# douglasbagnall/recur

Measured on AMD Instinct MI355X. Metric: BPTT timesteps*streams/sec at 1024-hidden/256-stream, higher is better.
Workload: dtype f32; 1 GPU; text-predict multi-tap generation: hidden 1024, 256 streams/GPU, BPTT depth 20, 42 symbols, RELU, weighted momentum, lr 1e-5; streams_per_gpu=256, global_streams=256, scaling_mode=weak, parallelism=single GPU, rccl_ranks=0, exchange=none

## Files before the change

### recur_amd/csrc/k_common.h

```cpp
#pragma once
#include <hip/hip_runtime.h>
#include <cstring>
#include <utility>
#include <type_traits>
#include <stdint.h>
#include <stdio.h>
#include <stdlib.h>
#include <math.h>
#include "ramd_internal.h"
#include "k_tiles.h"

#define HIP_CHECK(x)                                                              \
  do {                                                                            \
    hipError_t e_ = (x);                                                          \
    if (e_ != hipSuccess) {                                                       \
      fprintf(stderr, "librecur_amd: HIP error %s at %s:%d\n", hipGetErrorString(e_), \
              __FILE__, __LINE__);                                                \
      abort();                                                                    \
    }                                                                             \
  } while (0)

static inline void ramd_check_launch(const char *file, int line) {
  hipError_t e_ = hipGetLastError();
  if (e_ != hipSuccess) {
// ... 464 lines not shown
      const bool keep = s0 + i * 32 < hw.nrows && am[i] != 0;
#pragma unroll
      for (int rr = 0; rr < HO_HR; rr++) {
        const float x = keep ? hv[i][rr] : 0.0f;
        acc[rr].x += x * e4[i].x;
        acc[rr].y += x * e4[i].y;
        acc[rr].z += x * e4[i].z;
        acc[rr].w += x * e4[i].w;
      }
    }
  }
}
struct HoApply {
  float *w, *m;
  float rate, momentum, mw;
};
template <int HO_HR, int BATCH>
__device__ __forceinline__ void chain_ho_delta(const View &v, const HoWork &hw, float *lds, int rank, HoApply ap = HoApply{}) {
  const RamdShape &s = v.sh;
  const int H = s.H, O = s.O, OQ = O >> 2;
  const int HR = (H + hw.workers - 1) / hw.workers;
  const int tid = threadIdx.x, lane = tid & 63, wave = tid >> 6, q4 = lane & 15, gl = lane >> 4;
  const int h0 = rank * HR;
  float4 acc[HO_HR];
#pragma unroll
  for (int rr = 0; rr < HO_HR; rr++) acc[rr] = zero4();
  if (h0 < H) {
    const int q4c = q4 < OQ ? q4 : 0;
    if (hw.active) chain_ho_sum<true, HO_HR, BATCH>(v, hw, h0, HR, q4c, 4 * wave + gl, acc);
    else chain_ho_sum<false, HO_HR, BATCH>(v, hw, h0, HR, q4c, 4 * wave + gl, acc);
#pragma unroll
    for (int rr = 0; rr < HO_HR; rr++) {
      acc[rr].x += __shfl_xor(acc[rr].x, 16, 64); acc[rr].x += __shfl_xor(acc[rr].x, 32, 64);
      acc[rr].y += __shfl_xor(acc[rr].y, 16, 64); acc[rr].y += __shfl_xor(acc[rr].y, 32, 64);
      acc[rr].z += __shfl_xor(acc[rr].z, 16, 64); acc[rr].z += __shfl_xor(acc[rr].z, 32, 64);
      acc[rr].w += __shfl_xor(acc[rr].w, 16, 64); acc[rr].w += __shfl_xor(acc[rr].w, 32, 64);
    }
    if (gl == 0) {
#pragma unroll
      for (int rr = 0; rr < HO_HR; rr++) *reinterpret_cast<float4 *>(lds + 4 * ((wave * HO_HR + rr) * 16 + q4)) = acc[rr];
    }
  }
  const bool fin = tid < HO_HR * 16 && (tid >> 4) < HR && h0 + (tid >> 4) < H && (tid & 15) < OQ;
  const size_t fin_off = fin ? (size_t)(h0 + (tid >> 4)) * O + 4 * (tid & 15) : 0;
  float4 W4 = zero4(), M4 = zero4();
  if (fin && ap.w) {
    W4 = ld4(ap.w + fin_off);
    M4 = ld4(ap.m + fin_off);
  }
  __syncthreads();
  if (fin) {
    const int rr = tid >> 4, q = tid & 15;
    float4 sum = *reinterpret_cast<const float4 *>(lds + 4 * (rr * 16 + q));
    for (int w = 1; w < 8; w++) {
      const float4 t = *reinterpret_cast<const float4 *>(lds + 4 * ((w * HO_HR + rr) * 16 + q));
      sum.x += t.x; sum.y += t.y; sum.z += t.z; sum.w += t.w;
    }
    *reinterpret_cast<float4 *>(hw.dst + fin_off) = sum;
    if (ap.w) {
      float wv[4] = {W4.x, W4.y, W4.z, W4.w}, mv[4] = {M4.x, M4.y, M4.z, M4.w};
      const float dv[4] = {sum.x, sum.y, sum.z, sum.w};
#pragma unroll
      for (int i = 0; i < 4; i++) {
        const float t = dv[i] * ap.rate, mm = mv[i];
        wv[i] += t + mm * ap.mw;
        mv[i] = (mm + t) * ap.momentum;
      }
      *reinterpret_cast<float4 *>(ap.w + fin_off) = make_float4(wv[0], wv[1], wv[2], wv[3]);
      *reinterpret_cast<float4 *>(ap.m + fin_off) = make_float4(mv[0], mv[1], mv[2], mv[3]);
    }
  }
  __syncthreads();
}


struct XcWork {
  int on;
  int row0;
  int nx, nxp;
  const unsigned char *active;
  unsigned flags;
  int done;
  int dense;
};
RAMD_LOCAL int ramd_chain_steps(hipStream_t st, const View &v, const RamdShape *sh, const RamdBuffers *b,
                                int row0, int nrows, HoWork *ho, XcWork *xc);
```

### recur_amd/csrc/k_extras.h

```cpp
#pragma once
#include "k_common.h"
#ifndef XC_STAMP
#define XC_STAMP(i) do { } while (0)
#endif

template <int MAXQ> struct ExtrasIn {
  float4 ev[MAXQ];
  float xi, pv;
};
typedef unsigned u32x4_t __attribute__((ext_vector_type(4)));
template <int MAXQ>
__device__ __forceinline__ void extras_load(const View &v, int t, int r, int nx, int tn, int lane,
                                            ExtrasIn<MAXQ> &in) {
  const RamdShape &s = v.sh;
  const float *erow = v.b.ehi + (t * s.Scap + r) * s.I;
  const float *x = input_row_auto(v, r, t);
  const int nq = (s.H / 4 + 63) / 64;
  const int last4 = s.H / 4 - 1;
#pragma unroll
  for (int i = 0; i < MAXQ; i++) {
    const int k4 = lane + 64 * i;
    const float4 e = ld4(erow + 4 * min(k4, last4));
    in.ev[i] = (i < nq && k4 <= last4) ? e : zero4();
  }
// ... 127 lines not shown
  for (int k0 = 0; k0 < D; k0 += 64) {
    int k = k0 + lane;
    float es = (k < D) ? es_src[(size_t)k * es_stride] : 0.0f;
    bool stop = k < D && (es <= min_error_sum || es > max_error_sum);
    unsigned long long hit = __ballot(stop);
    int last = hit ? __ffsll((long long)hit) - 1 : min(63, D - 1 - k0);
    error_sum = __shfl(es, last, 64);
    if (hit) {
      n_exec = k0 + last + 1;
      break;
    }
  }
  bool broke = n_exec < D || (error_sum <= min_error_sum || error_sum > max_error_sum);
  int t = broke ? D - n_exec + 1 : 0;
  float scale;
  if (error_sum > error_sum_ceiling) {
    scale = soft_clip_dev(error_sum, max_error_sum);
  } else {
    scale = 1.0f;
    if (flags & 64u) {
      int depth_error = D / 4 - t;
      if (mef < MAX_MIN_ERROR_FACTOR_F && (min_error_gain != min_error_sum || depth_error < 0)) {
        mef = (float)((double)mef * (1.0 + depth_error * 1e-3));
      }
      mef = (mef >= ABS_MIN_ERROR_FACTOR_F) ? mef : ABS_MIN_ERROR_FACTOR_F;
    }
  }
  if (lane == 0) {
    as_global(v.b.mef)[r] = mef;
    as_global(v.b.ih_scale)[r] = scale;
    as_global(v.b.bptt_err)[r] = error_sum;
    as_global(v.b.n_exec)[r] = n_exec;
    as_global(v.b.depth_log)[r] = D - t;
    as_global(v.b.stat_depth)[r] = ci.depth_total + (double)(D - t);
  }
  const float cf = (flags & RAMD_IH_SCALE_IN_RATE) ? 1.0f : scale;
  for (int k = lane; k < D; k += 64) as_global(v.b.coef)[(size_t)k * s.Scap + r] = (k < n_exec) ? cf : 0.0f;
}


template <int MAXQ, int THREADS>
__device__ __forceinline__ void extras_control_stream(const View &v, int r, int j, int nx, int nxp, int tn,
                                                      const unsigned char *active, unsigned flags,
                                                      float *es_sh) {
  const RamdShape &s = v.sh;
  const int wave = threadIdx.x >> 6, lane = threadIdx.x & 63;
  const int items = tn == 0 ? s.D + 1 : s.D;
  float *hs_sh = es_sh + s.D;
  ExtrasIn<MAXQ> cur, nxt;
  ControlIn ci = {0.0f, 0.0f, 1.0f, 0.0, true};
  if (wave == 0) ci = bptt_control_load(v, r, j, active);
  if (wave < items) extras_load<MAXQ>(v, wave, r, nx, tn, lane, cur);
  for (int t = wave; t < items; t += THREADS / 64) {
    const int tnext = t + THREADS / 64;
    if (tnext < items) extras_load<MAXQ>(v, tnext, r, nx, tn, lane, nxt);
    if (tn == 0) {
      const float hs = row_sumsq<MAXQ>(cur);
      if (lane == 0) hs_sh[t] = hs;
    }
    if (t < s.D) {
      float es = extras_compute<MAXQ>(v, t, r, nx, nxp, tn, lane, cur);
      if (lane == 0) {
        if (tn != 0) v.b.esum[(size_t)t * s.Scap + r] = es;
        es_sh[t] = es;
      }
    }
    cur = nxt;
  }
  __syncthreads();
  if (wave == 0) {
    if (tn == 0) {
      for (int k = lane; k < s.D; k += 64) {
        const float es = hs_sh[k + 1] + es_sh[k];
        es_sh[k] = es;
        v.b.esum[(size_t)k * s.Scap + r] = es;
      }
      __builtin_amdgcn_s_waitcnt(0xc07f);
    }
    bptt_control_wave(v, r, j, lane, ci, flags, es_sh, 1);
  }
}

constexpr int XT_B = 3, XT_BL = 2;
struct TailPre {
  float xi[XT_B][2];
  ControlIn ci;
};
__device__ __forceinline__ void tail_items(int wave, int NW, int D, int &t0, int &stride, int &t_end) {
  const int NE = NW / 2;
  const int first_late = D > NE * XT_BL ? D - NE * XT_BL : 0;
  stride = NE;
  if (wave < NE) {
    t0 = wave;
    t_end = first_late;
  } else {
    t0 = first_late + (wave - NE);
    t_end = D;
  }
}
template <int THREADS>
__device__ __forceinline__ TailPre extras_tail_prefetch(const View &v, int r, int j, int nx, const unsigned char *active) {
  const RamdShape &s = v.sh;
  constexpr int NW = THREADS / 64;
  const int wave = __builtin_amdgcn_readfirstlane((int)(threadIdx.x >> 6)), lane = threadIdx.x & 63;
  const int D = s.D;
  TailPre p;
  p.ci = ControlIn{0.0f, 0.0f, 1.0f, 0.0, true};
  if (wave == 0) p.ci = bptt_control_load(v, r, j, active);
  const int xcol[2] = {(lane == 0 || lane >= nx) ? 0 : s.hidden_size + lane, lane + 64 < nx ? s.hidden_size + lane + 64 : 0};
  int t0, stride, t_end;
  tail_items(wave, NW, D, t0, stride, t_end);
#pragma unroll
  for (int b = 0; b < XT_B; b++) {
    const int t = t0 + stride * b;
    const auto *x = as_global(input_row<true>(v, r, t < D ? t : D - 1));
#pragma unroll
    for (int h = 0; h < 2; h++) p.xi[b][h] = x[xcol[h]];
  }
  return p;
}

template <int MAXQ, int THREADS, class WaitLast>
__device__ __forceinline__ void extras_control_tail(const View &v, int r, int j, int nx, int nxp,
                                                    const unsigned char *active, unsigned flags, float *es_sh,
                                                    const TailPre *pre, WaitLast &&wait_last) {
  constexpr int B = XT_B;
  const RamdShape &s = v.sh;
  constexpr int NW = THREADS / 64;
  const int wave = __builtin_amdgcn_readfirstlane((int)(threadIdx.x >> 6)), lane = threadIdx.x & 63;
  const int D = s.D;
  float *hs_sh = es_sh + D;
  const int nq = (s.H / 4 + 63) / 64, last4 = s.H / 4 - 1;
  ControlIn ci = {0.0f, 0.0f, 1.0f, 0.0, true};
  if (pre) ci = pre->ci;
  else if (wave == 0) ci = bptt_control_load(v, r, j, active);
  const __amdgpu_buffer_rsrc_t rs = __builtin_amdgcn_make_buffer_rsrc((void *)v.b.ehi, 0, 0x7fffffff, 0x00020000);
  const int xcol[2] = {(lane == 0 || lane >= nx) ? 0 : s.hidden_size + lane, lane + 64 < nx ? s.hidden_size + lane + 64 : 0};
  const unsigned xmask[2] = {lane < nx ? 0xffffffffu : 0u, lane + 64 < nx ? 0xffffffffu : 0u};
  unsigned koff[MAXQ];
  float km[MAXQ];
#pragma unroll
  for (int i = 0; i < MAXQ; i++) {
    const int k4 = lane + 64 * i;
    koff[i] = 16u * (unsigned)min(k4, last4);
    km[i] = (i < nq && k4 <= last4) ? 1.0f : 0.0f;
  }
  auto load_row = [&](int plane, float4 (&e)[MAXQ]) {
    const unsigned row_off = (unsigned)((plane * s.Scap + r) * s.I) * 4u;
#pragma unroll
    for (int i = 0; i < MAXQ; i++) {
      const u32x4_t q = __builtin_amdgcn_raw_buffer_load_b128(rs, (int)(row_off + koff[i]), 0, 16 );
      e[i] = make_float4(__uint_as_float(q.x), __uint_as_float(q.y), __uint_as_float(q.z), __uint_as_float(q.w));
    }
  };
  auto mask_row = [&](float4 (&e)[MAXQ]) {
#pragma unroll
    for (int i = 0; i < MAXQ; i++) { e[i].x *= km[i]; e[i].y *= km[i]; e[i].z *= km[i]; e[i].w *= km[i]; }
  };
  XC_STAMP(3);
  constexpr int NE = NW / 2;
  auto batch = [&](auto BC, const int tb, const int t_stride, const int t_end, const float (*xpre)[2]) {
    constexpr int BB = decltype(BC)::value;
    float xi[BB][2];
    float4 ev[BB][MAXQ], wh[BB][MAXQ], w0[MAXQ];
#pragma unroll
    for (int b = 0; b < BB; b++) {
      if (xpre) {
        xi[b][0] = __uint_as_float(__float_as_uint(xpre[b][0]) & xmask[0]);
        xi[b][1] = __uint_as_float(__float_as_uint(xpre[b][1]) & xmask[1]);
      } else {
        const int t = tb + t_stride * b;
        const auto *x = as_global(input_row<true>(v, r, t < D ? t : D - 1));
#pragma unroll
        for (int h = 0; h < 2; h++) xi[b][h] = __uint_as_float(__float_as_uint(x[xcol[h]]) & xmask[h]);
      }
    }
#pragma unroll
    for (int i = 0; i < MAXQ; i++) w0[i] = ld4g(reinterpret_cast<const char *>(v.b.ih_w) + koff[i]);
#pragma unroll
    for (int b = 0; b < BB; b++) {
      const int t = tb + t_stride * b;
      load_row(t < D ? t : D - 1, ev[b]);
    }
    XC_STAMP(5);
    unsigned long long live[BB][2];
    int l1[BB];
    auto value_of = [&](const float (&x)[2], int col) { return __shfl(col < 64 ? x[0] : x[1], col & 63, 64); };
#pragma unroll
    for (int b = 0; b < BB; b++) {
#pragma unroll
      for (int h = 0; h < 2; h++) live[b][h] = __ballot(act_live(s, xi[b][h]));
      const unsigned long long rest = live[b][0] & ~1ull;
      l1[b] = rest ? __ffsll((long long)rest) - 1 : live[b][1] ? 64 + __ffsll((long long)live[b][1]) - 1 : -1;
      const char *wr = reinterpret_cast<const char *>(v.b.ih_w + (size_t)(l1[b] >= 0 ? s.hidden_size + l1[b] : 0) * s.H);
#pragma unroll
      for (int i = 0; i < MAXQ; i++) wh[b][i] = ld4g(wr + koff[i]);
    }
    XC_STAMP(4);
    float hs[BB], a0[BB], a1[BB];
#pragma unroll
    for (int b = 0; b < BB; b++) {
      mask_row(ev[b]);
      hs[b] = a0[b] = a1[b] = 0.0f;
#pragma unroll
      for (int i = 0; i < MAXQ; i++) {
        const float4 e = ev[b][i];
        hs[b] += (e.x * e.x + e.y * e.y) + (e.z * e.z + e.w * e.w);
        a0[b] += e.x * w0[i].x + e.y * w0[i].y + e.z * w0[i].z + e.w * w0[i].w;
        a1[b] += e.x * wh[b][i].x + e.y * wh[b][i].y + e.z * wh[b][i].z + e.w * wh[b][i].w;
      }
    }
    for (int off = 32; off > 0; off >>= 1) {
#pragma unroll
      for (int b = 0; b < BB; b++) {
        hs[b] += __shfl_xor(hs[b], off, 64);
        a0[b] += __shfl_xor(a0[b], off, 64);
        a1[b] += __shfl_xor(a1[b], off, 64);
      }
    }
#pragma unroll
    for (int b = 0; b < BB; b++) {
      const int t = tb + t_stride * b;
      if (t >= t_end) continue;
      if (lane == 0) hs_sh[t] = hs[b];
      const bool has0 = (live[b][0] & 1ull) != 0;
      float e0 = has0 ? a0[b] : 0.0f, e1 = l1[b] >= 0 ? a1[b] : 0.0f;
      if (act_has_back_scale(s)) {
        e0 = resqrt_back_scale(value_of(xi[b], 0), e0);
        e1 = resqrt_back_scale(value_of(xi[b], l1[b] >= 0 ? l1[b] : 0), e1);
      }
      auto *dst = as_global(v.b.ex + ((size_t)(t + 1) * s.Scap + r) * nxp);
      if (lane < nx) dst[lane] = (lane == 0 && has0) ? e0 : (lane == l1[b]) ? e1 : 0.0f;
      if (lane + 64 < nx) dst[lane + 64] = (lane + 64 == l1[b]) ? e1 : 0.0f;
      float sq = 0.0f;
      if (has0) sq += e0 * e0;
      if (l1[b] >= 0) sq += e1 * e1;
      unsigned long long more[2] = {live[b][0] & ~1ull, live[b][1]};
      auto pop = [&]() {
        if (more[0]) {
          const int c = __ffsll((long long)more[0]) - 1;
          more[0] &= more[0] - 1;
          return c;
        }
        if (more[1]) {
          const int c = 64 + __ffsll((long long)more[1]) - 1;
          more[1] &= more[1] - 1;
          return c;
        }
        return -1;
      };
      (void)pop();
      while (more[0] | more[1]) {
        const int la = pop();
        const int lb = pop();
        const float xa = value_of(xi[b], la), xb = value_of(xi[b], lb >= 0 ? lb : la);
        const char *wa = reinterpret_cast<const char *>(v.b.ih_w + (size_t)(s.hidden_size + la) * s.H);
        const char *wb = reinterpret_cast<const char *>(v.b.ih_w + (size_t)(s.hidden_size + (lb >= 0 ? lb : la)) * s.H);
        float acca = 0.0f, accb = 0.0f;
#pragma unroll
        for (int i = 0; i < MAXQ; i++) {
          const float4 ta = ld4g(wa + koff[i]), tb4 = ld4g(wb + koff[i]);
          const float4 e = ev[b][i];
          acca += e.x * ta.x + e.y * ta.y + e.z * ta.z + e.w * ta.w;
          accb += e.x * tb4.x + e.y * tb4.y + e.z * tb4.z + e.w * tb4.w;
        }
        for (int off = 32; off > 0; off >>= 1) {
          acca += __shfl_xor(acca, off, 64);
          accb += __shfl_xor(accb, off, 64);
        }
        if (act_has_back_scale(s)) {
          acca = resqrt_back_scale(xa, acca);
          accb = resqrt_back_scale(xb, accb);
        }
        if (lane == 0) {
          dst[la] = acca;
          if (lb >= 0) dst[lb] = accb;
        }
        sq += acca * acca;
        if (lb >= 0) sq += accb * accb;
      }
      if (lane == 0) es_sh[t] = sq;
    }
    };
  constexpr int BL = XT_BL;
  const int first_late = D > NE * BL ? D - NE * BL : 0;
  if (wave < NE) {
    for (int tb = wave; tb < first_late; tb += NE * B)
      batch(std::integral_constant<int, B>{}, tb, NE, first_late, (pre && tb == wave) ? pre->xi : (const float (*)[2])nullptr);
  } else {
    float4 elast[MAXQ];
    if (wave == NW - 1) {
      wait_last();
      load_row(D, elast);
    }
    batch(std::integral_constant<int, BL>{}, first_late + (wave - NE), NE, D, pre ? pre->xi : (const float (*)[2])nullptr);
    if (wave == NW - 1) {
      mask_row(elast);
      float h = 0.0f;
#pragma unroll
      for (int i = 0; i < MAXQ; i++) h += (elast[i].x * elast[i].x + elast[i].y * elast[i].y) + (elast[i].z * elast[i].z + elast[i].w * elast[i].w);
      for (int off = 32; off > 0; off >>= 1) h += __shfl_xor(h, off, 64);
      if (lane == 0) hs_sh[D] = h;
    }
  }
  XC_STAMP(6);
  __syncthreads();
  XC_STAMP(7);
  if (wave == 0) {
    for (int k = lane; k < D; k += 64) {
      const float es = hs_sh[k + 1] + es_sh[k];
      es_sh[k] = es;
      as_global(v.b.esum)[(size_t)k * s.Scap + r] = es;
    }
    __builtin_amdgcn_s_waitcnt(0xc07f);
    bptt_control_wave(v, r, j, lane, ci, flags, es_sh, 1);
    XC_STAMP(8);
  }
}

template <int THREADS, class WaitLast>
__device__ __forceinline__ void extras_dense_tail(const View &v, int r, int j, int nx, int nxp, const unsigned char *active,
                                                  unsigned flags, float *lds, WaitLast &&wait_last) {
  constexpr int NW = THREADS / 64, NT3 = 3, PF = 4, LD = 16 * NT3 + 1;
  const RamdShape &s = v.sh;
  const int D = s.D;
  const int tid = threadIdx.x, wave = __builtin_amdgcn_readfirstlane((int)(threadIdx.x >> 6)), lane = tid & 63;
  const int lm = lane & 15, kq = lane >> 4;
  float *red = lds;
  float *rsq = red + NW * 32 * LD;
  float *rowsq = rsq + NW * 32;
  float *sqx = rowsq + 64;
  float *es_sh = sqx + 64;
  ControlIn ci = {0.0f, 0.0f, 1.0f, 0.0, true};
  if (wave == 0) ci = bptt_control_load(v, r, j, active);
  XC_STAMP(3);
  if (wave == NW - 1) wait_last();
  __syncthreads();
  XC_STAMP(5);
  const __amdgpu_buffer_rsrc_t rs = __builtin_amdgcn_make_buffer_rsrc((void *)v.b.ehi, 0, 0x7fffffff, 0x00020000);
  const float *brow[NT3];
#pragma unroll
  for (int jn = 0; jn < NT3; jn++) {
    const int c = 16 * jn + lm;
    brow[jn] = v.b.ih_w + (size_t)((c == 0 || c >= nx) ? 0 : s.hidden_size + c) * s.H;
  }
  const int nchunks = (s.H + 15) / 16;
  const int mine = (nchunks - wave + NW - 1) / NW;
  const float *xin0 = input_row<true>(v, r, 0);
  (void)xin0;
  for (int t0 = 0; t0 <= D; t0 += 32) {
    unsigned row_off[2];
#pragma unroll
    for (int i = 0; i < 2; i++) {
      const int t = min(t0 + 16 * i + lm, D);
      row_off[i] = (unsigned)((t * s.Scap + r) * s.I) * 4u;
    }
    f32x4 acc[2][NT3];
    float sq2[2] = {0.0f, 0.0f};
#pragma unroll
    for (int i = 0; i < 2; i++)
#pragma unroll
      for (int jn = 0; jn < NT3; jn++) acc[i][jn] = f32x4{0.f, 0.f, 0.f, 0.f};
    float4 fa[PF][2], fb[PF][NT3];
    float fm[PF];
    auto request = [&](int slot, int n) {
      const int k = 16 * (wave + NW * n) + 4 * kq;
      const bool in = n < mine && k < s.H;
      const int kc = in ? k : 0;
      fm[slot] = in ? 1.0f : 0.0f;
#pragma unroll
      for (int i = 0; i < 2; i++) {
        const u32x4_t q = __builtin_amdgcn_raw_buffer_load_b128(rs, (int)(row_off[i] + 4u * (unsigned)kc), 0, 16 );
        fa[slot][i] = make_float4(__uint_as_float(q.x), __uint_as_float(q.y), __uint_as_float(q.z), __uint_as_float(q.w));
      }
#pragma unroll
      for (int jn = 0; jn < NT3; jn++) fb[slot][jn] = ld4(brow[jn] + kc);
    };
#pragma unroll
// ... 95 lines not shown
```

### recur_amd/csrc/kernels_chain.hip

```cpp
#include "k_common.h"
#include "chain_plan.h"
#ifdef PC_STAMPS
__device__ unsigned long long g_xc_stamps[32];
#define XC_STAMP(i) do { if (blockIdx.x == 0 && threadIdx.x == ((i) == 10 ? 256 : 0)) g_xc_stamps[i] = __builtin_amdgcn_s_memrealtime(); } while (0)
#define PRO_STAMP(i, tid) do { if (blockIdx.x == PRO_WG && threadIdx.x == (tid)) g_xc_stamps[i] = __builtin_amdgcn_s_memrealtime(); } while (0)
#define PRO_STAMP_DEP(i, tid, dep) do { if (blockIdx.x == PRO_WG && threadIdx.x == (tid) && (dep) != 0x7ffffff1) g_xc_stamps[i] = __builtin_amdgcn_s_memrealtime(); } while (0)
#define PRO_CLOCKS(i, tid) do { if (blockIdx.x == PRO_WG && threadIdx.x == (tid)) { g_xc_stamps[i] = __builtin_amdgcn_s_memrealtime(); g_xc_stamps[(i) + 1] = __builtin_amdgcn_s_memtime(); } } while (0)
#ifndef PRO_WG
#define PRO_WG 0
#endif
#else
#define PRO_STAMP(i, tid) do { } while (0)
#define PRO_STAMP_DEP(i, tid, dep) do { } while (0)
#define PRO_CLOCKS(i, tid) do { } while (0)
#endif
#include "k_extras.h"
BND_DECL(g_bnd_chain, ramd_bnd_chain_stamps)


__global__ void k_store_view(View v, View *dst) { *dst = v; }

template <bool UNI, int NS = 0>
__global__ __launch_bounds__(512) void k_chain_main(const View *__restrict__ vp, int uniform_idx,
                                                    int row0, int nrows, int t, int tm, int tn,
// ... 274 lines not shown
      acc = __builtin_amdgcn_mfma_f32_32x32x2f32(a[u].z, b[u].z, acc, 0, 0, 0);
      acc = __builtin_amdgcn_mfma_f32_32x32x2f32(a[u].w, b[u].w, acc, 0, 0, 0);
    }
    __builtin_amdgcn_sched_barrier(0);
  };
  {
    f32x4 a0[NU], b0[NU], a1[NU], b1[NU];
    __builtin_amdgcn_s_barrier();
    rd(0, a0, b0);
#pragma unroll
    for (int st = 0; st < NS; st += 2) {
      step(st, a0, b0, a1, b1);
      if (st + 1 < NS) step(st + 1, a1, b1, a0, b0);
    }
  }
  float *red = wsm + (NS % W_STAGES) * W_STAGE_FLOATS;
#pragma unroll
  for (int g = 0; g < 16; g++) {
    const int row = wm * 32 + (g & 3) + 8 * (g >> 2) + 4 * kh;
    red[row * WN + wn * 32 + lm] = acc[g];
  }
  __syncthreads();
  float *dst0 = v.b.ehi + ((size_t)(t + 1) * s.Scap + row0 + m0) * s.I + n0 + c4;
#pragma unroll
  for (int rr = 0; rr < RPT; rr++) {
    const int row = RPT * rq + rr;
    float4 e4 = ld4(red + row * WN + c4);
    if (HALF) {
      const float4 f4 = ld4(red + (32 + row) * WN + c4);
      e4.x += f4.x;
      e4.y += f4.y;
      e4.z += f4.z;
      e4.w += f4.w;
    }
    const float e[4] = {e4.x, e4.y, e4.z, e4.w};
    float sq = 0.0f;
#pragma unroll
    for (int i = 0; i < 4; i++) {
      const float ev = act_backward(s, xin[rr][i], e[i]);
      dst0[(size_t)row * s.I + i] = ev;
      sq += ev * ev;
    }
    sq += __shfl_xor(sq, 1, 64);
    sq += __shfl_xor(sq, 2, 64);
    sq += __shfl_xor(sq, 4, 64);
    sq += __shfl_xor(sq, 8, 64);
    if ((etid & 15) == 0) v.b.esum_part[((size_t)t * (tn + 1) + nt) * s.Scap + row0 + m0 + row] = sq;
  }
}

constexpr int PC_SUB = 16;
constexpr int PC_RED_FLOATS = 4 * PC_SUB * 32;
constexpr int pc_lds_bytes(int K) { return (2 * PC_SUB * K + 2 * PC_RED_FLOATS) * 4 + 64; }
#ifndef PC_SLEEP0
#define PC_SLEEP0 22
#endif
#ifndef PC_SLEEP1
#define PC_SLEEP1 1
#endif
#ifndef PC_SLEEP0_ONE
#define PC_SLEEP0_ONE 12
#endif
#ifndef PC_SLEEP0_SMALL
#define PC_SLEEP0_SMALL 14
#endif
constexpr unsigned PC_EPOCH = 64;
#ifndef PC_POLL_SCALAR
#define PC_POLL_SCALAR 0
#endif
#ifndef PC_GAPS
#define PC_GAPS (PC_POLL_SCALAR ? 0x0 : 0x78)
#endif
#ifndef PC_GAPS_512
#define PC_GAPS_512 (PC_POLL_SCALAR ? 0x0 : 0x3c)
#endif
#ifndef PC_GAPS_256
#define PC_GAPS_256 (PC_POLL_SCALAR ? 0x0 : 0xe)
#endif
#ifndef PC_FILL_MFMAS
#define PC_FILL_MFMAS 0
#endif
#ifndef PC_FETCH_PRIO
#define PC_FETCH_PRIO 0
#endif
#ifndef PC_GAP_NOPS
#define PC_GAP_NOPS 0
#endif
typedef unsigned u32x8 __attribute__((ext_vector_type(8)));

struct ChainSync {
  unsigned tickets[8];
  unsigned pad0[24];
  unsigned flags[32][2][4][32];
  unsigned abort;
};
#define PC_SYNC_CLEAR_BYTES sizeof(ChainSync)
struct SeatTable {
  unsigned seat[8][256];
};
typedef const __attribute__((address_space(4))) unsigned *seat_tbl_p;
#define PC_HW_CU_KEY() (__builtin_amdgcn_s_getreg(((8 - 1) << 11) | (8 << 6) | 4) & 0xffu)

typedef __attribute__((address_space(1))) unsigned gu32;

#ifdef PC_STAMPS
__device__ unsigned long long g_pc_stamps[2][64][8];
#define PC_STAMP(role, k, slot)                                                                    \
  do {                                                                                             \
    if (g == 0 && j == 0 && lane == 0 && (wave8 & 3) == 0 && (k) < 64)                             \
      g_pc_stamps[role][k][slot] = __builtin_amdgcn_s_memrealtime();                               \
  } while (0)
#else
#define PC_STAMP(role, k, slot) do { } while (0)
#endif

#ifndef PC_ONE_SHARED_FETCH
#define PC_ONE_SHARED_FETCH 1
#endif
template <int ACT, int K, bool ONE = false, bool PAD = false, bool XD = false>
__global__ __launch_bounds__(512) void k_chain_persist(const View *__restrict__ vp, int uniform_idx,
                                                       int row0, int nrows, int depth, unsigned seq,
                                                       ChainSync *sy, unsigned *host_abort, int nvalid, int vlo,
                                                       HoWork hw, XcWork xc, int static_map, unsigned tseq, const unsigned *seats) {
  __builtin_amdgcn_s_setprio(2);
  const unsigned hw_xcc = __builtin_amdgcn_s_getreg((3 << 11) | (0 << 6) | 20) & 7u;
  const unsigned hw_seat = static_map == 2 ? ((seat_tbl_p)seats)[hw_xcc * 256u + PC_HW_CU_KEY()] : 0u;
  extern __shared__ __attribute__((aligned(16))) float psm[];
  constexpr int BUF = PC_SUB * K;
  constexpr int NT = K / 32;
  constexpr int KB = K / 64;
  constexpr int PPR = K / 256;
  float *abuf = psm;
  float *red = psm + 2 * BUF;
  unsigned *wg_info = reinterpret_cast<unsigned *>(red + 2 * PC_RED_FLOATS);
  XC_STAMP(0);
  BND_MARK(g_bnd_chain, 0);
  PRO_STAMP_DEP(16, 256, nrows);
  PRO_STAMP_DEP(17, 256, (int)hw_seat);
  View v = *vp;
  PRO_STAMP_DEP(18, 256, v.sh.H);
  v.b.uniform_idx = uniform_idx;
  const RamdShape &s = v.sh;
  const int wave8 = threadIdx.x >> 6, lane = threadIdx.x & 63;
  constexpr int TR = ONE ? PC_SUB : 2 * PC_SUB;
  const int mtiles = nrows / TR;

  unsigned seat, my_xcc;
  if (static_map == 2) {
    my_xcc = hw_xcc;
    seat = hw_seat;
  } else if (static_map) {
    my_xcc = blockIdx.x & 7u;
    seat = blockIdx.x >> 3;
    const unsigned real = __builtin_amdgcn_s_getreg((3 << 11) | (0 << 6) | 20) & 7u;
    if (real != my_xcc) seat = 32u;
  } else {
    if (threadIdx.x == 0) {
      const unsigned xcc = __builtin_amdgcn_s_getreg((3 << 11) | (0 << 6) | 20) & 7u;
      const unsigned t = __hip_atomic_fetch_add(&sy->tickets[xcc], 1u, __ATOMIC_RELAXED, __HIP_MEMORY_SCOPE_AGENT) -
                         (tseq - 1u) * 32u;
      wg_info[0] = xcc;
      wg_info[1] = t;
    }
    __syncthreads();
    seat = __builtin_amdgcn_readfirstlane(wg_info[1]);
    my_xcc = __builtin_amdgcn_readfirstlane(wg_info[0]);
  }
  const int g = (int)my_xcc + 8 * (int)(seat / NT);
  if (seat >= 32u) {
    if (threadIdx.x == 0) {
      __hip_atomic_store(&sy->abort, 1u, __ATOMIC_RELAXED, __HIP_MEMORY_SCOPE_AGENT);
      __hip_atomic_store(host_abort, 2u, __ATOMIC_RELAXED, __HIP_MEMORY_SCOPE_SYSTEM);
    }
    return;
  }
  if (g >= mtiles) {
    if (hw.dst && hw.idle_only) {
      constexpr int SP = 32 / NT;
      const int x = (int)my_xcc;
      auto r0 = [&](int xx) { const int r = (mtiles - xx + 7) / 8; return r < 0 ? 0 : r > SP ? SP : r; };
      int rank = (int)seat - r0(x) * NT;
      for (int xx = 0; xx < x; xx++) rank += (SP - r0(xx)) * NT;
      chain_ho_delta<9, 4>(v, hw, psm, rank);
    } else if (hw.dst) {
      chain_ho_delta<5, HO_BATCH>(v, hw, red, (int)blockIdx.x);
    }
    return;
  }
  const bool ho_here = hw.dst && !hw.idle_only;
  const int j = (int)(seat % NT);
  const int m0 = TR * g, n0 = 1 + 32 * j;
  const unsigned epoch0 = seq * PC_EPOCH;
  const int halfsteps = 2 * depth;
  const int tn = NT;
  const size_t plane_stride = (size_t)s.Scap * s.I;
  const bool xc_first = !XD && xc.on && j < TR && !(PAD && (m0 + j < vlo || m0 + j >= nvalid));
  TailPre tpre;
  PRO_STAMP(19, 256);
  if (xc_first) tpre = extras_tail_prefetch<512>(v, row0 + m0 + j, row0 + m0 + j - xc.row0, xc.nx, xc.active);
  PRO_STAMP(20, 256);

  if (wave8 >= 4) {
    const int wv = __builtin_amdgcn_readfirstlane(wave8) - 4, m = lane & 15, kq = lane >> 4;
    const int col = lane & 31, rh = lane >> 5;
    if (ho_here) chain_ho_delta<5, HO_BATCH>(v, hw, red, (int)blockIdx.x);
    PRO_STAMP(11, 256);
    float wreg[KB][4][2];
    {
      const float *wb = v.b.ih_w + (size_t)(n0 + m) * s.H + 1 + (K / 4) * wv + 4 * kq;
#pragma unroll
      for (int u = 0; u < KB; u++)
#pragma unroll
        for (int i = 0; i < 4; i++)
#pragma unroll
          for (int h = 0; h < 2; h++) wreg[u][i][h] = wb[(size_t)16 * h * s.H + 16 * u + i];
      PRO_STAMP(12, 256);
#pragma unroll
      for (int u = 0; u < KB; u++)
        asm volatile("" : : "v"(wreg[u][0][0]), "v"(wreg[u][0][1]), "v"(wreg[u][1][0]), "v"(wreg[u][1][1]),
                     "v"(wreg[u][2][0]), "v"(wreg[u][2][1]), "v"(wreg[u][3][0]), "v"(wreg[u][3][1]));
      PRO_STAMP(13, 256);
    }
    unsigned voff[2];
    bool mine[2][2];
#pragma unroll
    for (int q = 0; q < 2; q++) {
      voff[q] = (unsigned)(((size_t)(4 * wv + rh + 2 * q) * s.I + n0 + col) * sizeof(float));
#pragma unroll
      for (int x = 0; x < 2; x++) {
        const int sr = m0 + PC_SUB * x + 4 * wv + rh + 2 * q;
        mine[x][q] = !PAD || (sr >= vlo && sr < nvalid);
      }
    }
    const float *ehi_sub = v.b.ehi + (size_t)(row0 + m0) * s.I;
    unsigned hvoff[ONE ? 2 * PPR : 1];
    if constexpr (ONE) {
#pragma unroll
      for (int i = 0; i < 2 * PPR; i++) {
        const int ii = 2 * PPR + i, r = 4 * wv + ii / PPR;
        const int c = (64 * (ii % PPR) + lane) ^ r;
        hvoff[i] = (unsigned)(((size_t)r * s.I + 1 + 4 * c) * sizeof(float));
      }
    }
    uint32_t a_addr[2][4];
#pragma unroll
    for (int x = 0; x < 2; x++)
#pragma unroll
      for (int i = 0; i < 4; i++)
        a_addr[x][i] = lds_byte_addr(abuf + x * BUF + m * K) + 16u * (uint32_t)((K / 16) * wv + ((4 * i + kq) ^ m));
    const uint32_t red_rd = lds_byte_addr(red) + 4u * (uint32_t)((4 * wv + rh) * 32 + col);
    float xg0 = 0.f, xg1 = 0.f;
    f32x4 af[4];
    bool mdead = false;
    __syncthreads();
    PRO_STAMP(14, 256);
    PRO_CLOCKS(24, 256);

    auto half = [&](auto XC, const int k) -> bool {
      constexpr int x = decltype(XC)::value, xf = x ^ 1;
      const bool multiplies = k < halfsteps && !(ONE && x == 1);
      PC_STAMP(0, k, 0);
      if (multiplies) {
        af[0] = lds_read_b128_off<0>(a_addr[x][0]);
        if (KB > 1) af[1] = lds_read_b128_off<0>(a_addr[x][1]);
        if (KB > 2) af[2] = lds_read_b128_off<0>(a_addr[x][2]);
      }
      if (k >= 1 && !(ONE && x == 0)) {
        const int t = (k - 1) >> 1;
        float ev[2];
        asm volatile("s_waitcnt vmcnt(0)" : "+v"(xg0), "+v"(xg1));
        {
          const uint32_t ra = red_rd + 4u * (uint32_t)(xf * PC_RED_FLOATS);
          float p[2][4];
#pragma unroll
          for (int q = 0; q < 2; q++) {
            p[q][0] = q ? lds_read_b32_off<256 + 0 * 2048>(ra) : lds_read_b32_off<0 * 2048>(ra);
            p[q][1] = q ? lds_read_b32_off<256 + 1 * 2048>(ra) : lds_read_b32_off<1 * 2048>(ra);
            p[q][2] = q ? lds_read_b32_off<256 + 2 * 2048>(ra) : lds_read_b32_off<2 * 2048>(ra);
            p[q][3] = q ? lds_read_b32_off<256 + 3 * 2048>(ra) : lds_read_b32_off<3 * 2048>(ra);
// ... 85 lines not shown
          __builtin_amdgcn_s_sleep(1);
#endif
          __builtin_amdgcn_sched_barrier(0);
        }
      });
      {
        float *rdw = red + x * PC_RED_FLOATS + wv * (PC_SUB * 32);
#pragma unroll
        for (int r = 0; r < 4; r++) {
          rdw[(4 * kq + r) * 32 + m] = acc0[r];
          rdw[(4 * kq + r) * 32 + 16 + m] = acc1[r];
        }
      }
      PC_STAMP(0, k, 1);
      __syncthreads();
      return true;
    };
    for (int k = 0;; k += 2) {
      if (!half(std::integral_constant<int, 0>{}, k)) break;
      if (!half(std::integral_constant<int, 1>{}, k + 1)) break;
    }
  } else {
  const int lw = __builtin_amdgcn_readfirstlane(wave8);
  const int col = lane & 31, rh = lane >> 5;
  gu32 *aborted = (gu32 *)&sy->abort;
  bool dead = false;

  unsigned voff[4 * PPR];
#pragma unroll
  for (int i = 0; i < 4 * PPR; i++) {
    const int r = 4 * lw + i / PPR;
    const int c = (64 * (i % PPR) + lane) ^ r;
    voff[i] = (unsigned)(((size_t)r * s.I + 1 + 4 * c) * sizeof(float));
  }
  const float *sub_base = v.b.ehi + (size_t)(row0 + m0) * s.I;
  auto fetch = [&](int x, int plane, bool first_half_only = false) {
    const char *base = reinterpret_cast<const char *>(sub_base + (size_t)plane * plane_stride +
                                                      (size_t)x * PC_SUB * s.I);
    const uint32_t dst = __builtin_amdgcn_readfirstlane(lds_byte_addr(abuf + x * BUF + 4 * lw * K));
#pragma unroll
    for (int i = 0; i < 4 * PPR; i++)
      if (i < 2 * PPR || !first_half_only)
        lds_dma16_sc1(base, voff[i], dst + (uint32_t)(((i / PPR) * K + 256 * (i % PPR)) * sizeof(float)));
  };
  const unsigned poll_off = (unsigned)((lane % NT) * sizeof(unsigned));
  auto give_up = [&]() {
    if (lane == 0) {
      __hip_atomic_store(aborted, 1u, __ATOMIC_RELAXED, __HIP_MEMORY_SCOPE_AGENT);
      __hip_atomic_store(host_abort, 1u, __ATOMIC_RELAXED, __HIP_MEMORY_SCOPE_SYSTEM);
    }
    dead = true;
  };
  auto wait_for = [&](int x, int t) {
    const unsigned want = epoch0 + (unsigned)t + 1u;
    const unsigned *fbase = &sy->flags[g][x][lw][0];
    __builtin_amdgcn_s_sleep(ONE ? PC_SLEEP0_ONE : K == 1024 ? PC_SLEEP0 : PC_SLEEP0_SMALL);
    for (unsigned spins = 0;; spins++) {
#if PC_POLL_SCALAR
      unsigned behind = 0u;
#pragma unroll
      for (int i = 0; i < NT / 8; i++) {
        u32x8 f;
        asm volatile("s_load_dwordx8 %0, %1, %2 glc\n\ts_waitcnt lgkmcnt(0)" : "=s"(f) : "s"(fbase), "n"(32 * i) : "memory");
#pragma unroll
        for (int e = 0; e < 8; e++) behind |= (f[e] - want) >> 31;
      }
      if (!behind) return;
#else
      unsigned got;
      asm volatile("global_load_dword %0, %1, %2 sc1\n\ts_waitcnt vmcnt(0)" : "=v"(got) : "v"(poll_off), "s"(fbase) : "memory");
      if (__all(got >= want)) return;
#endif
      if ((spins & 1023u) == 1023u) {
        const unsigned ab = __hip_atomic_load(aborted, __ATOMIC_RELAXED, __HIP_MEMORY_SCOPE_AGENT);
        if (__any(ab != 0u) || spins > (1u << 21)) {
          give_up();
          return;
        }
      }
      __builtin_amdgcn_s_sleep(PC_SLEEP1);
    }
  };

  fetch(0, 0);
  if (halfsteps > 1 && !ONE) fetch(1, 0);
  if (ho_here) chain_ho_delta<5, HO_BATCH>(v, hw, red, (int)blockIdx.x);
  asm volatile("s_waitcnt vmcnt(0)" ::: "memory");
  PRO_STAMP(15, 0);
  __syncthreads();
  for (int k = 0; k < halfsteps; k++) {
    PC_STAMP(1, k, 0);
    if (k >= 1 && k + 1 < halfsteps && !dead && !(ONE && (k & 1) == 0)) {
      wait_for((k - 1) & 1, (k - 1) >> 1);
      PC_STAMP(1, k, 2);
#if PC_FETCH_PRIO
      __builtin_amdgcn_s_setprio(3);
#endif
      if (!dead) fetch((k + 1) & 1, (k + 1) >> 1, ONE && PC_ONE_SHARED_FETCH);
#if PC_FETCH_PRIO
      __builtin_amdgcn_s_setprio(0);
#endif
      PC_STAMP(1, k, 3);
    }
    asm volatile("s_waitcnt vmcnt(0)" ::: "memory");
    PC_STAMP(1, k, 4);
    __syncthreads();
  }
  }

  if (!xc.on) return;
  XC_STAMP(1);
  XC_STAMP(10);
  PRO_CLOCKS(26, 256);
  for (int i = j; i < TR; i += NT) {
    const int sr = m0 + i;
    if (PAD && (sr < vlo || sr >= nvalid)) continue;
    const int x = i / PC_SUB, rg = (i % PC_SUB) >> 2;
    auto wait_last = [&]() {
      const unsigned want = epoch0 + (unsigned)depth;
      const char *fbase = uniform_ptr(&sy->flags[g][x][rg][0]);
      const unsigned poff = (unsigned)((lane % NT) * sizeof(unsigned));
      for (unsigned spins = 0;; spins++) {
        unsigned got;
        asm volatile("global_load_dword %0, %1, %2 sc1\n\ts_waitcnt vmcnt(0)" : "=v"(got) : "v"(poff), "s"(fbase) : "memory");
        if (__all(got >= want)) break;
        if ((spins & 1023u) == 1023u) {
          const unsigned ab = __hip_atomic_load((gu32 *)&sy->abort, __ATOMIC_RELAXED, __HIP_MEMORY_SCOPE_AGENT);
          if (__any(ab != 0u) || spins > (1u << 21)) {
            if (lane == 0) {
              __hip_atomic_store((gu32 *)&sy->abort, 1u, __ATOMIC_RELAXED, __HIP_MEMORY_SCOPE_AGENT);
              __hip_atomic_store(host_abort, 1u, __ATOMIC_RELAXED, __HIP_MEMORY_SCOPE_SYSTEM);
            }
            break;
          }
        }
        __builtin_amdgcn_s_sleep(PC_SLEEP1);
      }
      XC_STAMP(2);
    };
    constexpr int XQ = (K / 4 + 1 + 63) / 64;
    const int r = row0 + sr;
    if constexpr (XD)
      extras_dense_tail<512>(v, r, r - xc.row0, xc.nx, xc.nxp, xc.active, xc.flags, abuf, wait_last);
    else
      extras_control_tail<XQ, 512>(v, r, r - xc.row0, xc.nx, xc.nxp, xc.active, xc.flags, abuf, (i == j && xc_first) ? &tpre : nullptr, wait_last);
    XC_STAMP(9);
    __syncthreads();
  }
  BND_MARK(g_bnd_chain, 1);
}

const View *device_view(hipStream_t st, const View &v) {
  static View *d_view = nullptr;
  static View h_view;
  static bool have = false;
  View cur = v;
  cur.b.uniform_idx = 0;
  cur.b.noise_spec = nullptr;
  cur.b.rng_spec = nullptr;
  cur.b.noise_spec_use = 0;
  cur.b.dense_inputs = 0;
  if (!d_view) HIP_CHECK(hipMalloc(&d_view, sizeof(View)));
  if (!have || memcmp(&cur, &h_view, sizeof(View)) != 0) {
    RAMD_LAUNCH(k_store_view, dim3(1), dim3(1), 0, st, cur, d_view);
    h_view = cur;
    have = true;
  }
  return d_view;
}

static bool g_chain_validated = false, g_chain_broken = false, g_xcd_static = false, g_seat_table = false;
static unsigned *g_seats = nullptr;

struct ProbeOut {
  unsigned arrived, fail;
  unsigned xcc[256];
  unsigned cu_key[256];
};
__global__ __launch_bounds__(512) void k_residency_probe(ProbeOut *p) {
  extern __shared__ float probe_lds[];
  if (threadIdx.x != 0) return;
  p->xcc[blockIdx.x] = __builtin_amdgcn_s_getreg((3 << 11) | (0 << 6) | 20) & 7u;
  p->cu_key[blockIdx.x] = PC_HW_CU_KEY();
  __hip_atomic_fetch_add(&p->arrived, 1u, __ATOMIC_RELAXED, __HIP_MEMORY_SCOPE_AGENT);
  for (unsigned spins = 0; __hip_atomic_load(&p->arrived, __ATOMIC_RELAXED, __HIP_MEMORY_SCOPE_AGENT) < gridDim.x; spins++) {
    if (spins > (1u << 20) || __hip_atomic_load(&p->fail, __ATOMIC_RELAXED, __HIP_MEMORY_SCOPE_AGENT)) {
      __hip_atomic_store(&p->fail, 1u, __ATOMIC_RELAXED, __HIP_MEMORY_SCOPE_AGENT);
      return;
    }
    __builtin_amdgcn_s_sleep(8);
  }
}

#ifdef PC_STAMPS
extern "C" void ramd_chain_stamps(unsigned long long *out) {
  HIP_CHECK(hipDeviceSynchronize());
  HIP_CHECK(hipMemcpyFromSymbol(out, HIP_SYMBOL(g_pc_stamps), sizeof(unsigned long long) * 2 * 64 * 8));
}
extern "C" void ramd_chain_tail_stamps(unsigned long long *out) {
  HIP_CHECK(hipDeviceSynchronize());
  HIP_CHECK(hipMemcpyFromSymbol(out, HIP_SYMBOL(g_xc_stamps), sizeof(unsigned long long) * 32));
}
#endif

static ChainSync *g_chain_sync = nullptr;
static unsigned *g_chain_abort_host = nullptr, *g_chain_abort_dev = nullptr;
static unsigned g_chain_seq = 0;
static int g_chain_cus = -1;
static void chain_validate(hipStream_t st) {
  if (g_chain_validated || g_chain_broken) return;
  if (g_chain_cus < 0) {
    int dev = 0;
    hipDeviceProp_t prop;
    HIP_CHECK(hipGetDevice(&dev));
    HIP_CHECK(hipGetDeviceProperties(&prop, dev));
    g_chain_cus = prop.multiProcessorCount;
  }
  if (g_chain_cus != 256) {
    g_chain_broken = true;
    return;
  }
  if (!g_chain_sync) {
    HIP_CHECK(hipMalloc(&g_chain_sync, sizeof(ChainSync)));
    HIP_CHECK(hipMemset(g_chain_sync, 0, PC_SYNC_CLEAR_BYTES));
    ramd_abort_word_dev();
  }
  ProbeOut *d_probe = nullptr, h_probe;
  HIP_CHECK(hipMalloc(&d_probe, sizeof(ProbeOut)));
// ... 28 lines not shown
          const unsigned t = keys[c];
          keys[c] = keys[c - 1];
          keys[c - 1] = t;
        }
      for (int a = 0; a < n && ok; a++) {
        if (a > 0 && keys[a] == keys[a - 1]) ok = false;
        tbl[x][keys[a]] = (unsigned)a;
      }
    }
    g_seat_table = ok && env_int("RECUR_AMD_XCD_TABLE", 1);
    if (g_seat_table) {
      if (!g_seats) HIP_CHECK(hipMalloc(&g_seats, sizeof(SeatTable)));
      HIP_CHECK(hipMemcpy(g_seats, &h_seats, sizeof(SeatTable), hipMemcpyHostToDevice));
    }
  }
  g_chain_validated = true;
}

static bool g_side_streams = false;
static unsigned g_ticket_launches = 0;
extern "C" void ramd_note_side_stream(void) { g_side_streams = true; }

extern "C" unsigned *ramd_abort_word_dev(void) {
  if (!g_chain_abort_host) {
    HIP_CHECK(hipHostMalloc((void **)&g_chain_abort_host, 64, hipHostMallocMapped));
    *g_chain_abort_host = 0;
    HIP_CHECK(hipHostGetDevicePointer((void **)&g_chain_abort_dev, g_chain_abort_host, 0));
  }
  return g_chain_abort_dev;
}

extern "C" unsigned ramd_chain_abort_word(void) {
  return g_chain_abort_host ? *(volatile unsigned *)g_chain_abort_host : 0u;
}


static bool chain_available(hipStream_t st) {
  chain_validate(st);
  return g_chain_validated && !g_chain_broken;
}

struct PersistLaunch {
  hipStream_t st;
  const View *d_view;
  int uniform_idx, D;
  ChainSegment s;
  unsigned seq;
  HoWork hw;
  XcWork xc;
};

template <int ACT, int K, bool ONE, bool PAD, bool XD> static void launch_persist(const PersistLaunch &c) {
  const int use_static = g_seat_table ? 2 : (g_xcd_static && !g_side_streams) ? 1 : 0;
  const unsigned tseq = use_static ? 0u : ++g_ticket_launches;
  raise_lds_limit<k_chain_persist<ACT, K, ONE, PAD, XD>>(pc_lds_bytes(K));
  RAMD_LAUNCH((k_chain_persist<ACT, K, ONE, PAD, XD>), dim3(256), dim3(512), pc_lds_bytes(K), c.st, c.d_view, c.uniform_idx,
              c.s.row0, c.s.nrows, c.D, c.seq, g_chain_sync, g_chain_abort_dev, c.s.nvalid, c.s.vlo, c.hw, c.xc, use_static, tseq,
              g_seats);
}
template <int ACT, int K, bool XD> static void launch_persist_tiles(const PersistLaunch &c) {
  if (c.s.pad) launch_persist<ACT, K, true, true, XD>(c);
  else if (c.s.one) launch_persist<ACT, K, true, false, XD>(c);
  else launch_persist<ACT, K, false, false, XD>(c);
}
template <int ACT, int K> static void launch_persist_tail(const PersistLaunch &c) {
  if constexpr (K >= 512)
    if (c.xc.on && c.xc.dense) return launch_persist_tiles<ACT, K, true>(c);
  launch_persist_tiles<ACT, K, false>(c);
}
template <int ACT> static void launch_persist_k(const PersistLaunch &c, int hidden_size) {
  switch (hidden_size) {
  case 1024: return launch_persist_tail<ACT, 1024>(c);
  case 512: return launch_persist_tail<ACT, 512>(c);
  default: return launch_persist_tail<ACT, 256>(c);
  }
}

static bool launch_chain_persist(hipStream_t st, const View *d_view, const RamdShape *sh, const RamdBuffers *b,
                                 const ChainSegment &s, HoWork *ho, XcWork *xcp) {
  PersistLaunch c = {st, d_view, b->uniform_idx, sh->D, s, 0u, {}, {}};
  const int test_giveup = env_int("RECUR_AMD_CHAIN_TEST_GIVEUP", 0);
  const bool checked = env_int("RECUR_AMD_CHAIN_CHECK", 0) || test_giveup > 1;
  if (xcp && !checked) c.xc = *xcp;
  if (xcp && !c.xc.on) xcp->on = 0;
  if (ho && !ho->done) {
    c.hw = *ho;
    c.hw.workers = s.workers, c.hw.idle_only = s.idle_only;
  }
  if (g_chain_seq >= (1u << 25)) {
    HIP_CHECK(hipStreamSynchronize(st));
    HIP_CHECK(hipMemset(g_chain_sync, 0, PC_SYNC_CLEAR_BYTES));
    g_chain_seq = 0;
    g_ticket_launches = 0;
  }
  c.seq = ++g_chain_seq;
  int ev = timing_begin(st, T_CHAIN, 1);
  if (sh->activation == 2) launch_persist_k<2>(c, sh->hidden_size);
  else if (sh->activation == 5) launch_persist_k<5>(c, sh->hidden_size);
  else launch_persist_k<1>(c, sh->hidden_size);
  timing_end(st, ev);
  if (checked) {
    static int checked_launches = 0;
    HIP_CHECK(hipStreamSynchronize(st));
    const unsigned word = *(volatile unsigned *)g_chain_abort_host;
    if (word || ++checked_launches == test_giveup) {
      fprintf(stderr, "librecur_amd: a one-launch BPTT chain gave up in mid-run (code %u: its 256 workgroups were no longer "
                      "all resident, or a hand-off timed out); this call's chain runs again a launch per step, which is "
                      "what the process uses from here on\n", word);
      *(volatile unsigned *)g_chain_abort_host = 0;
      HIP_CHECK(hipMemset(g_chain_sync, 0, PC_SYNC_CLEAR_BYTES));
      g_chain_seq = 0;
      g_ticket_launches = 0;
      g_chain_broken = true;
      return false;
    }
  }
  if (ho && c.hw.dst) ho->done = 1;
  return true;
}

struct StepsLaunch {
  hipStream_t st;
  const View *d_view;
  int uniform_idx, row0, nrows, D;
  ChainSteps f;
};
template <int NS, int MT> static void launch_wide_steps(const StepsLaunch &c) {
  const size_t shm = (size_t)W_STAGES * W_STAGE_FLOATS * sizeof(float);
  raise_lds_limit<k_chain_wide<NS, MT>>((int)shm);
  for (int t = 0; t < c.D; t++)
    RAMD_LAUNCH((k_chain_wide<NS, MT>), dim3(c.f.blocks), dim3(512), shm, c.st, c.d_view, c.uniform_idx, c.row0, c.nrows, t,
                c.f.tm, c.f.tn);
}
template <int NS> static void launch_wide_mt(const StepsLaunch &c) {
  if (c.f.mt == 32) launch_wide_steps<NS, 32>(c);
  else launch_wide_steps<NS, 64>(c);
}
template <bool UNI, int NS> static void launch_main_steps(const StepsLaunch &c) {
  for (int t = 0; t < c.D; t++)
    RAMD_LAUNCH((k_chain_main<UNI, NS>), dim3(c.f.blocks), dim3(512), 0, c.st, c.d_view, c.uniform_idx, c.row0, c.nrows, t,
                c.f.tm, c.f.tn, c.f.nstages);
}
static void launch_chain_steps(const StepsLaunch &c) {
  int ev = timing_begin(c.st, T_CHAIN, c.D);
  const int ns = c.f.ns;
  if (c.f.form == CHAIN_WIDE) {
    if (ns == 32) launch_wide_mt<32>(c);
    else if (ns == 24) launch_wide_mt<24>(c);
    else launch_wide_mt<16>(c);
  } else if (!c.f.uniform) launch_main_steps<false, 0>(c);
  else if (ns == 16) launch_main_steps<true, 16>(c);
  else if (ns == 8) launch_main_steps<true, 8>(c);
  else if (ns == 4) launch_main_steps<true, 4>(c);
  else if (ns == 2) launch_main_steps<true, 2>(c);
  else launch_main_steps<true, 0>(c);
  timing_end(c.st, ev);
}

int ramd_chain_steps(hipStream_t st, const View &v, const RamdShape *sh, const RamdBuffers *b, int row0,
                     int nrows, HoWork *ho, XcWork *xc) {
  const View *d_view = device_view(st, v);
  const bool available = chain_persist_wanted(sh, b, row0, nrows) && chain_available(st);
  const ChainPlan p = ramd_plan_chain(sh, b, row0, nrows, available);
  bool persist = p.seg_rows > 0;
  ChainSegment s;
  for (int r = 0; persist && chain_segment(p, r, &s); r += s.nrows) persist = launch_chain_persist(st, d_view, sh, b, s, ho, xc);
// ... 8 lines not shown
```

Measured before the change: 1.224 million stream-timesteps/s.

## Park early-wave tail ehi rows in LDS during final chain half-step

During the last half-step of the persistent chain kernel, the early waves DMA their first batch of ehi rows for the extras control tail into the spare LDS operand buffer. The tail then reads that first batch from LDS instead of global memory, hiding load latency behind the chain's final step. This adds a sleep and extra DMA traffic in the last half-step, and reuses the operand buffer region, which relies on its layout. It is enabled by default through an environment flag.

Result: no change. 1.228 million stream-timesteps/s, median of 6 (+0.3%).

```diff
diff --git a/recur_amd/csrc/k_common.h b/recur_amd/csrc/k_common.h
--- a/recur_amd/csrc/k_common.h
+++ b/recur_amd/csrc/k_common.h
@@ -570,6 +570,7 @@
   unsigned flags;
   int done;
   int dense;
+  int park;
 };
 RAMD_LOCAL int ramd_chain_steps(hipStream_t st, const View &v, const RamdShape *sh, const RamdBuffers *b,
                                 int row0, int nrows, HoWork *ho, XcWork *xc);
diff --git a/recur_amd/csrc/k_extras.h b/recur_amd/csrc/k_extras.h
--- a/recur_amd/csrc/k_extras.h
+++ b/recur_amd/csrc/k_extras.h
@@ -233,6 +233,7 @@
 }
 
 constexpr int XT_B = 3, XT_BL = 2;
+constexpr int TAIL_PARK_ROW = 5 * 1024, TAIL_PARK_OFF = 4096, TAIL_PARK_SLOTS = 4 * XT_B;
 struct TailPre {
   float xi[XT_B][2];
   ControlIn ci;
@@ -271,10 +272,11 @@
   return p;
 }
 
-template <int MAXQ, int THREADS, class WaitLast>
+template <int MAXQ, int THREADS, bool PK = false, class WaitLast>
 __device__ __forceinline__ void extras_control_tail(const View &v, int r, int j, int nx, int nxp,
                                                     const unsigned char *active, unsigned flags, float *es_sh,
-                                                    const TailPre *pre, WaitLast &&wait_last) {
+                                                    const TailPre *pre, WaitLast &&wait_last, uint32_t parked = 0u) {
+  static_assert(!PK || (THREADS == 512 && MAXQ == 5), "parked rows: four early waves, 257 float4 per row");
   constexpr int B = XT_B;
   const RamdShape &s = v.sh;
   constexpr int NW = THREADS / 64;
@@ -310,8 +312,9 @@
   };
   XC_STAMP(3);
   constexpr int NE = NW / 2;
-  auto batch = [&](auto BC, const int tb, const int t_stride, const int t_end, const float (*xpre)[2]) {
+  auto batch = [&](auto BC, auto LC, const int tb, const int t_stride, const int t_end, const float (*xpre)[2]) {
     constexpr int BB = decltype(BC)::value;
+    constexpr bool from_lds = decltype(LC)::value;
     float xi[BB][2];
     float4 ev[BB][MAXQ], wh[BB][MAXQ], w0[MAXQ];
 #pragma unroll
@@ -331,7 +334,16 @@
 #pragma unroll
     for (int b = 0; b < BB; b++) {
       const int t = tb + t_stride * b;
-      load_row(t < D ? t : D - 1, ev[b]);
+      if constexpr (from_lds) {
+        typedef const __attribute__((address_space(3))) f32x4 *lds4_p;
+#pragma unroll
+        for (int i = 0; i < MAXQ; i++) {
+          const f32x4 q = *(lds4_p)(parked + (uint32_t)(t * TAIL_PARK_ROW) + koff[i]);
+          ev[b][i] = make_float4(q.x, q.y, q.z, q.w);
+        }
+      } else {
+        load_row(t < D ? t : D - 1, ev[b]);
+      }
     }
     XC_STAMP(5);
     unsigned long long live[BB][2];
@@ -436,15 +448,22 @@
   constexpr int BL = XT_BL;
   const int first_late = D > NE * BL ? D - NE * BL : 0;
   if (wave < NE) {
-    for (int tb = wave; tb < first_late; tb += NE * B)
-      batch(std::integral_constant<int, B>{}, tb, NE, first_late, (pre && tb == wave) ? pre->xi : (const float (*)[2])nullptr);
+    int tb = wave;
+    if constexpr (PK) {
+      if (parked != 0u && tb < first_late) {
+        batch(std::integral_constant<int, B>{}, std::true_type{}, tb, NE, first_late, pre ? pre->xi : (const float (*)[2])nullptr);
+        tb += NE * B;
+      }
+    }
+    for (; tb < first_late; tb += NE * B)
+      batch(std::integral_constant<int, B>{}, std::false_type{}, tb, NE, first_late, (pre && tb == wave) ? pre->xi : (const float (*)[2])nullptr);
   } else {
     float4 elast[MAXQ];
     if (wave == NW - 1) {
       wait_last();
       load_row(D, elast);
     }
-    batch(std::integral_constant<int, BL>{}, first_late + (wave - NE), NE, D, pre ? pre->xi : (const float (*)[2])nullptr);
+    batch(std::integral_constant<int, BL>{}, std::false_type{}, first_late + (wave - NE), NE, D, pre ? pre->xi : (const float (*)[2])nullptr);
     if (wave == NW - 1) {
       mask_row(elast);
       float h = 0.0f;
diff --git a/recur_amd/csrc/kernels_chain.hip b/recur_amd/csrc/kernels_chain.hip
--- a/recur_amd/csrc/kernels_chain.hip
+++ b/recur_amd/csrc/kernels_chain.hip
@@ -380,6 +380,9 @@
 #endif
 #ifndef PC_FETCH_PRIO
 #define PC_FETCH_PRIO 0
+#endif
+#ifndef PC_PARK_SLEEP
+#define PC_PARK_SLEEP 16
 #endif
 #ifndef PC_GAP_NOPS
 #define PC_GAP_NOPS 0
@@ -493,6 +496,9 @@
   const int tn = NT;
   const size_t plane_stride = (size_t)s.Scap * s.I;
   const bool xc_first = !XD && xc.on && j < TR && !(PAD && (m0 + j < vlo || m0 + j >= nvalid));
+  constexpr bool PARKS = !XD && K == 1024 && !ONE;
+  static_assert(!PARKS || TAIL_PARK_OFF + TAIL_PARK_SLOTS * TAIL_PARK_ROW <= BUF * (int)sizeof(float), "the parked rows lie in sub-chain a's operand buffer");
+  const bool park_on = PARKS && xc.park && xc_first;
   TailPre tpre;
   PRO_STAMP(19, 256);
   if (xc_first) tpre = extras_tail_prefetch<512>(v, row0 + m0 + j, row0 + m0 + j - xc.row0, xc.nx, xc.active);
@@ -744,6 +750,28 @@
     }
   };
 
+  unsigned pk_voff = 0u;
+  if constexpr (PARKS) {
+    pk_voff = 16u * (unsigned)lane;
+    asm volatile("" : "+v"(pk_voff));
+  }
+  auto park = [&]() {
+    int t0, t_stride, t_end;
+    tail_items(lw, 8, depth, t0, t_stride, t_end);
+    const char *row = uniform_ptr(sub_base + (size_t)j * s.I);
+    const uint32_t dst = __builtin_amdgcn_readfirstlane(lds_byte_addr(abuf)) + (uint32_t)TAIL_PARK_OFF;
+#pragma unroll
+    for (int b = 0; b < XT_B; b++) {
+      const int t = t0 + t_stride * b;
+      if (t < t_end) {
+        const char *src = row + (size_t)t * plane_stride * sizeof(float);
+#pragma unroll
+        for (int i = 0; i < TAIL_PARK_ROW / 1024; i++)
+          lds_dma16_sc1(src + 1024 * i, pk_voff, dst + (uint32_t)(t * TAIL_PARK_ROW + 1024 * i));
+      }
+    }
+  };
+
   fetch(0, 0);
   if (halfsteps > 1 && !ONE) fetch(1, 0);
   if (ho_here) chain_ho_delta<5, HO_BATCH>(v, hw, red, (int)blockIdx.x);
@@ -763,6 +791,13 @@
       __builtin_amdgcn_s_setprio(0);
 #endif
       PC_STAMP(1, k, 3);
+    }
+    if constexpr (PARKS) {
+      if (park_on && k + 1 == halfsteps) {
+        __builtin_amdgcn_s_sleep(PC_PARK_SLEEP);
+        park();
+        PC_STAMP(1, k, 3);
+      }
     }
     asm volatile("s_waitcnt vmcnt(0)" ::: "memory");
     PC_STAMP(1, k, 4);
@@ -805,7 +840,8 @@
     if constexpr (XD)
       extras_dense_tail<512>(v, r, r - xc.row0, xc.nx, xc.nxp, xc.active, xc.flags, abuf, wait_last);
     else
-      extras_control_tail<XQ, 512>(v, r, r - xc.row0, xc.nx, xc.nxp, xc.active, xc.flags, abuf, (i == j && xc_first) ? &tpre : nullptr, wait_last);
+      extras_control_tail<XQ, 512, PARKS>(v, r, r - xc.row0, xc.nx, xc.nxp, xc.active, xc.flags, abuf, (i == j && xc_first) ? &tpre : nullptr, wait_last,
+                                          (i == j && park_on) ? lds_byte_addr(abuf) + (uint32_t)TAIL_PARK_OFF : 0u);
     XC_STAMP(9);
     __syncthreads();
   }
@@ -1000,6 +1036,7 @@
   const int test_giveup = env_int("RECUR_AMD_CHAIN_TEST_GIVEUP", 0);
   const bool checked = env_int("RECUR_AMD_CHAIN_CHECK", 0) || test_giveup > 1;
   if (xcp && !checked) c.xc = *xcp;
+  c.xc.park = env_int("RECUR_AMD_TAIL_PARK", 1) != 0;
   if (xcp && !c.xc.on) xcp->on = 0;
   if (ho && !ho->done) {
     c.hw = *ho;
```
